# Borda/pyImSegm

Measured on NVIDIA H100. Metric: megapixels/sec end-to-end SLIC+features+GC (pipe_color2d_slic_features_model_graphcut), higher is better.
Workload: dtype f64

## Files before the change

pyimsegm_b200/csrc/graph.cu:

```cuda
#include "common.cuh"
#include <cooperative_groups.h>
namespace cg = cooperative_groups;

namespace {


struct AdjWs {
    unsigned long long* table;
    int* deg;
    int* off;
    int* fill;
    int* tmp_a;
    int* ctr;
    int slots;
};

__device__ __forceinline__ unsigned hash64(unsigned long long k)
{
    k ^= k >> 33; k *= 0xff51afd7ed558ccdull; k ^= k >> 33; k *= 0xc4ceb9fe1a85ec53ull; k ^= k >> 33;
    return (unsigned)k;
}

__device__ void edge_insert(const AdjWs& w, int l0, int l1)
{
// ... 160 lines not shown
    cg::cluster_group cl = cg::this_cluster();
    if (threadIdx.x == 0) *s_x = t;
    cl.sync();
    double tot = is_max ? -1.0 : 0.0;
    for (int r = 0; r < ECL; ++r) { const double pr = *cl.map_shared_rank(s_x, r); tot = is_max ? fmax(tot, pr) : tot + pr; }
    cl.sync();
    return tot;
}

__global__ void __cluster_dims__(ECL, 1, 1) __launch_bounds__(1024) k_gc_energies(const double* __restrict__ proba, int N_in, const int* n_nodes_dev, int K, const int* __restrict__ edges, int E_in,
                                                      const int* n_edges_dev, const double* __restrict__ centres,
                                                      const double* __restrict__ vfeat, int D, int metric, int spatial,
                                                      double edge_cost, const double* __restrict__ pairwise, double* unary,
                                                      double* edge_w, int* unary_i, int* edge_wi, int* smooth_i, double* sp)
{
    __shared__ double s_red[32];
    __shared__ double s_x;
    const int tid = blockIdx.x * blockDim.x + threadIdx.x, nth = gridDim.x * blockDim.x;
    const int E = n_edges_dev ? (*n_edges_dev > E_in ? 0 : *n_edges_dev) : E_in;
    const int N = n_nodes_dev ? min(*n_nodes_dev, N_in) : N_in;
    double umax = 0.0;
    for (int i = tid; i < N * K; i += nth) {
        double p = proba[i];
        if (p < 0.01) p = 0.01;
        if (p > 1.0 - 0.01) p = 1.0 - 0.01;
        double u = fabs(-log(p));
        unary[i] = u;
        umax = fmax(umax, fabs(u));
    }
    umax = cluster_reduce(umax, true, s_red, &s_x);
    double dsum = 0.0, ssum = 0.0;
    for (int e = tid; e < E; e += nth) {
        int a = edges[2 * e], b = edges[2 * e + 1];
        double dist = 0.0;
        if (metric != 0) {
            const double* va = vfeat + (size_t)a * D;
            const double* vb = vfeat + (size_t)b * D;
            for (int k = 0; k < D; ++k) {
                double df = va[k] - vb[k];
                if (metric == 1) dist = fmax(dist, df * df);
                else if (metric == 2) dist += fabs(df);
                else dist += df * df;
            }
            if (metric == 3) dist = sqrt(dist);
        }
        edge_w[e] = dist;
        dsum += dist;
        if (spatial) {
            double cy = centres[2 * a] - centres[2 * b], cx = centres[2 * a + 1] - centres[2 * b + 1];
            double s = sqrt(cy * cy + cx * cx);
            sp[e] = s;
            ssum += s;
        }
    }
    dsum = cluster_reduce(dsum, false, s_red, &s_x);
    ssum = cluster_reduce(ssum, false, s_red, &s_x);
    const double dmean = E > 0 ? dsum / E : 0.0, smean = E > 0 ? ssum / E : 1.0;
    double vsum = 0.0;
    if (metric != 0)
        for (int e = tid; e < E; e += nth) { double t = edge_w[e] - dmean; vsum += t * t; }
    vsum = cluster_reduce(vsum, false, s_red, &s_x);
    const double sd = sqrt(E > 0 ? vsum / E : 0.0);
    const double denom = 2.0 * (sd * sd);
    double wmax = 0.0;
    for (int e = tid; e < E; e += nth) {
        double wv = metric != 0 ? exp(-edge_w[e] / denom) : 1.0;
        if (spatial) wv = wv / (sp[e] / smean);
        if (wv < 1e-3) wv = 1e-3;
        if (wv > 1e3) wv = 1e3;
        wv *= edge_cost;
        edge_w[e] = wv;
        wmax = fmax(wmax, fabs(wv));
    }
    wmax = cluster_reduce(wmax, true, s_red, &s_x);
    double pmax = pairwise[0];
    for (int i = 1; i < K * K; ++i) pmax = fmax(pmax, pairwise[i]);
    const double dwf = fmax(umax, wmax * pmax) + 1e-10;
    for (int i = tid; i < N * K; i += nth) unary_i[i] = (int)((unary[i] / dwf) * 100000.0);
    for (int e = tid; e < E; e += nth) edge_wi[e] = (int)((edge_w[e] / dwf) * 1000.0);
    for (int i = tid; i < K * K; i += nth) smooth_i[i] = (int)(pairwise[i] * 100.0);
}


__global__ void __launch_bounds__(256) k_gather(const int* __restrict__ seg, long long n, const int* __restrict__ lut_i,
                                                const double* __restrict__ lut_p, int K, int* __restrict__ out_i, double* __restrict__ out_p)
{
    long long p = (long long)blockIdx.x * blockDim.x + threadIdx.x;
    if (p >= n) return;
    int l = seg[p];
    if (out_i) out_i[p] = lut_i[l];
    if (out_p) {
        const double* src = lut_p + (size_t)l * K;
        double* dst = out_p + (size_t)p * K;
        for (int k = 0; k < K; ++k) dst[k] = src[k];
    }
}

}

extern "C" size_t isb_adjacency_workspace_bytes(int nb, int cap)
{
    AdjWs w;
    return carve_adj(w, nullptr, 0, nb, cap);
}

extern "C" int isb_adjacency_edges(const int32_t* seg, int H, int W, int nb, int32_t* edges, int cap, int32_t* n_edges_out, void* ws,
                                   size_t ws_bytes, isb_stream_t stream)
{
    ISB_REQUIRE(seg && edges && n_edges_out && ws, "null pointer");
    ISB_REQUIRE(H > 0 && W > 0 && nb > 0 && cap > 0, "bad sizes");
    AdjWs w;
    size_t need = carve_adj(w, ws, ws_bytes, nb, cap);
    ISB_REQUIRE(need <= ws_bytes, "workspace too small");
    cudaStream_t st = (cudaStream_t)stream;
    ProfScope prof(ISB_PROF_ADJ, st);
    ISB_CUDA_CHECK(cudaMemsetAsync(w.table, 0xFF, sizeof(unsigned long long) * (size_t)w.slots, st));
    ISB_CUDA_CHECK(cudaMemsetAsync(w.deg, 0, sizeof(int) * (size_t)nb, st));
    ISB_CUDA_CHECK(cudaMemsetAsync(w.ctr, 0, sizeof(int) * 4, st));
    size_t n = (size_t)H * W;
    k_edge_scan<<<(unsigned)((n + 255) / 256), 256, 0, st>>>(seg, H, W, w);
    ISB_LAUNCH_CHECK();
    k_edge_offsets<<<1, 1024, 0, st>>>(nb, w, cap, n_edges_out);
    ISB_LAUNCH_CHECK();
    k_edge_fill<<<(w.slots + 255) / 256, 256, 0, st>>>(w, cap);
    ISB_LAUNCH_CHECK();
    k_edge_emit<<<(nb + 127) / 128, 128, 0, st>>>(nb, w, cap, edges);
    ISB_LAUNCH_CHECK();
    return ISB_OK;
}

extern "C" int isb_adjacency_edges_3d(const int32_t* seg, int D, int H, int W, int nb, int32_t* edges, int cap, int32_t* n_edges_out,
                                      void* ws, size_t ws_bytes, isb_stream_t stream)
{
    ISB_REQUIRE(seg && edges && n_edges_out && ws, "null pointer");
    ISB_REQUIRE(D > 0 && H > 0 && W > 0 && nb > 0 && cap > 0, "bad sizes");
    AdjWs w;
    size_t need = carve_adj(w, ws, ws_bytes, nb, cap);
    ISB_REQUIRE(need <= ws_bytes, "workspace too small");
    cudaStream_t st = (cudaStream_t)stream;
    ProfScope prof(ISB_PROF_ADJ, st);
    ISB_CUDA_CHECK(cudaMemsetAsync(w.table, 0xFF, sizeof(unsigned long long) * (size_t)w.slots, st));
    ISB_CUDA_CHECK(cudaMemsetAsync(w.deg, 0, sizeof(int) * (size_t)nb, st));
    ISB_CUDA_CHECK(cudaMemsetAsync(w.ctr, 0, sizeof(int) * 4, st));
    size_t n = (size_t)D * H * W;
    k_edge_scan3d<<<(unsigned)((n + 255) / 256), 256, 0, st>>>(seg, D, H, W, w);
    ISB_LAUNCH_CHECK();
    k_edge_offsets<<<1, 1024, 0, st>>>(nb, w, cap, n_edges_out);
    ISB_LAUNCH_CHECK();
    k_edge_fill<<<(w.slots + 255) / 256, 256, 0, st>>>(w, cap);
    ISB_LAUNCH_CHECK();
    k_edge_emit<<<(nb + 127) / 128, 128, 0, st>>>(nb, w, cap, edges);
    ISB_LAUNCH_CHECK();
    return ISB_OK;
}

extern "C" int isb_centroids_3d(const int32_t* seg, int D, int H, int W, int nb, double* centres, void* ws, size_t ws_bytes, isb_stream_t stream)
{
    ISB_REQUIRE(seg && centres && ws, "null pointer");
    ISB_REQUIRE(D > 0 && H > 0 && W > 0 && nb > 0, "bad sizes");
    ISB_REQUIRE(ws_bytes >= sizeof(unsigned long long) * 4 * (size_t)nb, "workspace too small (4 * nb uint64)");
    cudaStream_t st = (cudaStream_t)stream;
    ISB_CUDA_CHECK(cudaMemsetAsync(ws, 0, sizeof(unsigned long long) * 4 * (size_t)nb, st));
    size_t n = (size_t)D * H * W;
    k_centroid3d_acc<<<(unsigned)((n + 255) / 256), 256, 0, st>>>(seg, D, H, W, (unsigned long long*)ws);
    ISB_LAUNCH_CHECK();
    k_centroid3d_fin<<<(nb + 255) / 256, 256, 0, st>>>(nb, (const unsigned long long*)ws, centres);
    ISB_LAUNCH_CHECK();
    return ISB_OK;
}

extern "C" size_t isb_gc_energies_workspace_bytes(int N, int K, int E) { return isb_align(sizeof(double) * (size_t)(E > 0 ? E : 1)); }

extern "C" int isb_gc_energies(const double* proba, int N, const int32_t* n_nodes_dev, int K, const int32_t* edges, int E, const int32_t* n_edges_dev,
                               const double* centres, int metric, int spatial, double edge_cost, const double* pairwise, double* unary,
                               double* edge_w, int32_t* unary_i, int32_t* edge_wi, int32_t* smooth_i, void* ws, size_t ws_bytes,
                               isb_stream_t stream)
{
    ISB_REQUIRE(proba && edges && pairwise && unary && edge_w && unary_i && edge_wi && smooth_i && ws, "null pointer");
    ISB_REQUIRE(N > 0 && K > 0 && E >= 0, "bad sizes");
    ISB_REQUIRE(metric >= 0 && metric <= 3, "metric must be 0..3");
    ISB_REQUIRE(!spatial || centres, "centres are required for spatially normalised edge weights");
    ISB_REQUIRE(ws_bytes >= isb_gc_energies_workspace_bytes(N, K, E), "workspace too small");
    ProfScope prof(ISB_PROF_ENERGY, (cudaStream_t)stream);
    k_gc_energies<<<ECL, 1024, 0, (cudaStream_t)stream>>>(proba, N, n_nodes_dev, K, edges, E, n_edges_dev, centres, proba, K, metric, spatial, edge_cost,
                                                         pairwise, unary, edge_w, unary_i, edge_wi, smooth_i, (double*)ws);
    ISB_LAUNCH_CHECK();
    return ISB_OK;
}

__global__ void k_fill_i32(int* p, long long n, int v)
{
    long long i = (long long)blockIdx.x * blockDim.x + threadIdx.x;
    if (i < n) p[i] = v;
}

extern "C" int isb_fill_i32(int32_t* dst, long long n, int32_t value, isb_stream_t stream)
{
    ISB_REQUIRE(dst && n > 0, "bad arguments");
    k_fill_i32<<<(unsigned)((n + 255) / 256), 256, 0, (cudaStream_t)stream>>>(dst, n, value);
    ISB_LAUNCH_CHECK();
    return ISB_OK;
}

__global__ void k_combine(void* dst, const void* src, long long n, int op)
{
    long long i = (long long)blockIdx.x * blockDim.x + threadIdx.x;
    if (i >= n) return;
    if (op == 0) ((long long*)dst)[i] += ((const long long*)src)[i];
    else if (op == 1) { long long a = ((long long*)dst)[i], b = ((const long long*)src)[i]; ((long long*)dst)[i] = a > b ? a : b; }
    else if (op == 2) ((double*)dst)[i] = fmin(((double*)dst)[i], ((const double*)src)[i]);
    else if (op == 3) ((double*)dst)[i] = fmax(((double*)dst)[i], ((const double*)src)[i]);
    else ((double*)dst)[i] = ((double*)dst)[i] + ((const double*)src)[i];
}

extern "C" int isb_combine(void* dst, const void* src, long long n, int op, isb_stream_t stream)
{
    ISB_REQUIRE(dst && src && n > 0 && op >= 0 && op <= 4, "bad arguments");
    k_combine<<<(unsigned)((n + 255) / 256), 256, 0, (cudaStream_t)stream>>>(dst, src, n, op);
    ISB_LAUNCH_CHECK();
    return ISB_OK;
}

extern "C" int isb_gather(const int32_t* seg, long long npx, const int32_t* lut_i, const double* lut_p, int K, int32_t* out_i,
                          double* out_p, isb_stream_t stream)
{
    ISB_REQUIRE(seg && npx > 0, "bad arguments");
    ISB_REQUIRE((!out_i || lut_i) && (!out_p || (lut_p && K > 0)), "LUT missing for a requested output");
    ProfScope prof(ISB_PROF_GATHER, (cudaStream_t)stream);
    k_gather<<<(unsigned)((npx + 255) / 256), 256, 0, (cudaStream_t)stream>>>(seg, npx, lut_i, lut_p, K, out_i, out_p);
    ISB_LAUNCH_CHECK();
    return ISB_OK;
}
```

pyimsegm_b200/csrc/segment_stats.cu:

```cuda
#include "common.cuh"

namespace {

constexpr int SROWS = 16;

struct StatWs {
    double* acc;
    double* var;
    long long* iacc;
    float* meanf;
};

__device__ __forceinline__ float clean(float v) { return isnan(v) ? 0.0f : v; }

__global__ void __launch_bounds__(256) k_stats_pass1(const void* __restrict__ img, int dtype, const int* __restrict__ seg, int H, int W,
                                                     int y_off, StatWs ws)
{
    const int x = blockIdx.x * 256 + threadIdx.x;
    if (x >= W) return;
    const int y0 = blockIdx.y * SROWS, y1 = min(y0 + SROWS, H);
    int cur = -1;
    double s0 = 0, s1 = 0, s2 = 0, e0 = 0, e1 = 0, e2 = 0;
    long long cnt = 0, sy = 0;
    for (int y = y0; y <= y1; ++y) {
        int l = -1;
        float v0 = 0, v1 = 0, v2 = 0;
        if (y < y1) {
            size_t p = (size_t)y * W + x;
            l = seg[p];
            if (img) {
                v0 = clean(load_as_f32(img, dtype, 3 * p));
                v1 = clean(load_as_f32(img, dtype, 3 * p + 1));
                v2 = clean(load_as_f32(img, dtype, 3 * p + 2));
            }
        }
        if (l != cur) {
            if (cur >= 0) {
                double* a = ws.acc + 6 * (size_t)cur;
                atomicAdd(a, s0); atomicAdd(a + 1, s1); atomicAdd(a + 2, s2);
                atomicAdd(a + 3, e0); atomicAdd(a + 4, e1); atomicAdd(a + 5, e2);
                unsigned long long* ia = (unsigned long long*)(ws.iacc + 3 * (size_t)cur);
                atomicAdd(ia, (unsigned long long)cnt);
                atomicAdd(ia + 1, (unsigned long long)sy);
                atomicAdd(ia + 2, (unsigned long long)(cnt * x));
            }
            cur = l;
            s0 = s1 = s2 = e0 = e1 = e2 = 0;
            cnt = 0; sy = 0;
        }
        if (y < y1) {
            s0 += (double)v0; s1 += (double)v1; s2 += (double)v2;
            e0 += (double)__fmul_rn(v0, v0); e1 += (double)__fmul_rn(v1, v1); e2 += (double)__fmul_rn(v2, v2);
            cnt += 1; sy += y + y_off;
        }
    }
}

__global__ void k_stats_means(int nb, StatWs ws)
{
    int k = blockIdx.x * blockDim.x + threadIdx.x;
    if (k >= nb) return;
    long long c = ws.iacc[3 * (size_t)k];
    for (int z = 0; z < 3; ++z) {
        double m = ws.acc[6 * (size_t)k + z];
        if (c > 0) m = m / (double)c;
        ws.meanf[3 * (size_t)k + z] = (float)m;
    }
}

__global__ void __launch_bounds__(256) k_stats_pass2(const void* __restrict__ img, int dtype, const int* __restrict__ seg, int H, int W,
                                                     StatWs ws)
{
    const int x = blockIdx.x * 256 + threadIdx.x;
    if (x >= W) return;
    const int y0 = blockIdx.y * SROWS, y1 = min(y0 + SROWS, H);
    int cur = -1;
    double a0 = 0, a1 = 0, a2 = 0;
    float m0 = 0, m1 = 0, m2 = 0;
    for (int y = y0; y <= y1; ++y) {
        int l = -1;
        size_t p = (size_t)y * W + x;
        if (y < y1) l = seg[p];
        if (l != cur) {
            if (cur >= 0) {
                double* a = ws.var + 3 * (size_t)cur;
                atomicAdd(a, a0); atomicAdd(a + 1, a1); atomicAdd(a + 2, a2);
            }
            cur = l;
            a0 = a1 = a2 = 0;
            if (l >= 0) { m0 = ws.meanf[3 * (size_t)l]; m1 = ws.meanf[3 * (size_t)l + 1]; m2 = ws.meanf[3 * (size_t)l + 2]; }
        }
        if (y < y1) {
            float d0 = __fsub_rn(clean(load_as_f32(img, dtype, 3 * p)), m0);
            float d1 = __fsub_rn(clean(load_as_f32(img, dtype, 3 * p + 1)), m1);
            float d2 = __fsub_rn(clean(load_as_f32(img, dtype, 3 * p + 2)), m2);
            a0 += (double)__fmul_rn(d0, d0); a1 += (double)__fmul_rn(d1, d1); a2 += (double)__fmul_rn(d2, d2);
        }
    }
}

__device__ __forceinline__ double tidy(double v)
{
    if (isnan(v)) return 0.0;
    if (isinf(v)) return v > 0 ? 1.7976931348623157e308 : -1.7976931348623157e308;
    return v == 0.0 ? 0.0 : v;
}

__global__ void k_stats_finalize(int nb, int flags, StatWs ws, double* feat, int ld, int col0, double* centres, int* counts)
{
    int k = blockIdx.x * blockDim.x + threadIdx.x;
    if (k >= nb) return;
    long long c = ws.iacc[3 * (size_t)k];
    double dn = (double)c;
    int col = col0;
    double* row = feat ? feat + (size_t)k * ld : nullptr;
    if (row) {
        if (flags & 1) { for (int z = 0; z < 3; ++z) { double v = ws.acc[6 * (size_t)k + z]; if (c > 0) v = v / dn; row[col++] = tidy(v); } }
        if (flags & 2) { for (int z = 0; z < 3; ++z) { double v = ws.var[3 * (size_t)k + z]; if (c > 0) v = v / dn; row[col++] = tidy(sqrt(v)); } }
        if (flags & 4) { for (int z = 0; z < 3; ++z) { double v = ws.acc[6 * (size_t)k + 3 + z]; if (c > 0) v = v / dn; row[col++] = tidy(v); } }
    }
    if (centres) {
        if (c > 0) { centres[2 * (size_t)k] = (double)ws.iacc[3 * (size_t)k + 1] / dn; centres[2 * (size_t)k + 1] = (double)ws.iacc[3 * (size_t)k + 2] / dn; }
        else { centres[2 * (size_t)k] = -1.0; centres[2 * (size_t)k + 1] = -1.0; }
    }
    if (counts) counts[k] = (int)c;
}

static size_t carve(StatWs& w, void* ws, size_t bytes, int nb)
{
    WsCarver c(ws, bytes);
    w.acc = c.take<double>(6 * (size_t)nb);
    w.var = c.take<double>(3 * (size_t)nb);
    w.iacc = c.take<long long>(3 * (size_t)nb);
    w.meanf = c.take<float>(3 * (size_t)nb);
    return isb_align(c.off);
}

}

extern "C" size_t isb_segment_stats_workspace_bytes(int nb)
{
    StatWs w;
    return carve(w, nullptr, 0, nb);
}

extern "C" int isb_segment_stats_2d(const void* img, int dtype, const int32_t* seg, int H, int W, int nb, int flags, double* feat,
                                    int ld, int col0, double* centres, int32_t* counts, void* ws, size_t ws_bytes,
                                    isb_stream_t stream)
{
    ISB_REQUIRE(seg && ws && (img || (flags & 7) == 0), "null pointer");
    ISB_REQUIRE(H > 0 && W > 0 && nb > 0, "bad sizes");
    ISB_REQUIRE(dtype >= ISB_U8 && dtype <= ISB_F64, "bad dtype");
    StatWs w;
    size_t need = carve(w, ws, ws_bytes, nb);
    ISB_REQUIRE(need <= ws_bytes, "workspace too small");
    cudaStream_t st = (cudaStream_t)stream;
    ProfScope prof(ISB_PROF_STATS, st);
    ISB_CUDA_CHECK(cudaMemsetAsync(ws, 0, need, st));
    dim3 grid((W + 255) / 256, (H + SROWS - 1) / SROWS);
    k_stats_pass1<<<grid, 256, 0, st>>>(img, dtype, seg, H, W, 0, w);
    ISB_LAUNCH_CHECK();
    if (flags & 2) {
        k_stats_means<<<(nb + 255) / 256, 256, 0, st>>>(nb, w);
        ISB_LAUNCH_CHECK();
        k_stats_pass2<<<grid, 256, 0, st>>>(img, dtype, seg, H, W, w);
        ISB_LAUNCH_CHECK();
    }
    k_stats_finalize<<<(nb + 255) / 256, 256, 0, st>>>(nb, flags, w, feat, ld, col0, centres, counts);
    ISB_LAUNCH_CHECK();
    return ISB_OK;
}


extern "C" int isb_segment_stats_accumulate(const void* img, int dtype, const int32_t* seg, int H, int W, int y_off, int nb, double* acc,
                                            int64_t* iacc, isb_stream_t stream)
{
    ISB_REQUIRE(seg && acc && iacc, "null pointer");
    ISB_REQUIRE(H > 0 && W > 0 && nb > 0 && y_off >= 0, "bad sizes");
    ISB_REQUIRE(dtype >= ISB_U8 && dtype <= ISB_F64, "bad dtype");
    cudaStream_t st = (cudaStream_t)stream;
    ProfScope prof(ISB_PROF_STATS, st);
    StatWs w;
    w.acc = acc; w.iacc = (long long*)iacc; w.var = nullptr; w.meanf = nullptr;
    dim3 grid((W + 255) / 256, (H + SROWS - 1) / SROWS);
    k_stats_pass1<<<grid, 256, 0, st>>>(img, dtype, seg, H, W, y_off, w);
    ISB_LAUNCH_CHECK();
    return ISB_OK;
}

extern "C" int isb_segment_stats_deviation(const void* img, int dtype, const int32_t* seg, int H, int W, int nb, const double* acc,
                                           const int64_t* iacc, float* meanf_scratch, double* var, isb_stream_t stream)
{
    ISB_REQUIRE(img && seg && acc && iacc && meanf_scratch && var, "null pointer");
    ISB_REQUIRE(H > 0 && W > 0 && nb > 0, "bad sizes");
    ISB_REQUIRE(dtype >= ISB_U8 && dtype <= ISB_F64, "bad dtype");
    cudaStream_t st = (cudaStream_t)stream;
    ProfScope prof(ISB_PROF_STATS, st);
    StatWs w;
    w.acc = (double*)acc; w.iacc = (long long*)iacc; w.var = var; w.meanf = meanf_scratch;
    k_stats_means<<<(nb + 255) / 256, 256, 0, st>>>(nb, w);
    ISB_LAUNCH_CHECK();
    dim3 grid((W + 255) / 256, (H + SROWS - 1) / SROWS);
    k_stats_pass2<<<grid, 256, 0, st>>>(img, dtype, seg, H, W, w);
    ISB_LAUNCH_CHECK();
    return ISB_OK;
}

extern "C" int isb_segment_stats_finish(int nb, int flags, const double* acc, const double* var, const int64_t* iacc, double* feat, int ld,
                                        int col0, double* centres, int32_t* counts, isb_stream_t stream)
{
    ISB_REQUIRE(acc && iacc && (var || !(flags & 2)), "null pointer");
    ISB_REQUIRE(nb > 0, "bad sizes");
    cudaStream_t st = (cudaStream_t)stream;
    StatWs w;
    w.acc = (double*)acc; w.iacc = (long long*)iacc; w.var = (double*)var; w.meanf = nullptr;
    k_stats_finalize<<<(nb + 255) / 256, 256, 0, st>>>(nb, flags, w, feat, ld, col0, centres, counts);
    ISB_LAUNCH_CHECK();
    return ISB_OK;
}
```

pyimsegm_b200/csrc/slic_connectivity.cu:

```cuda
#include "common.cuh"

namespace {

struct ConnWs {
    int* comp;
    int* size;
    int* aux;
    int* queue;
    int* list;
    int* row_cnt;
    int* ctr;
    int4* bbox;
};

constexpr int VISBIT = 1 << 30;
__device__ __forceinline__ int dec(int c) { return (c < 0 ? ~c : c) & ~VISBIT; }

__device__ __forceinline__ int find_root(const int* parent, int i)
{
    while (true) {
        int p = parent[i];
        if (p == i) return i;
        i = p;
    }
}

__device__ __forceinline__ void unite(int* parent, int a, int b)
{
    while (true) {
        a = find_root(parent, a);
        b = find_root(parent, b);
        if (a == b) return;
        if (a < b) { int t = a; a = b; b = t; }
        int old = atomicMin(&parent[a], b);
        if (old == a) return;
        a = old;
    }
}

__global__ void __launch_bounds__(256) k_row_runs(const int* __restrict__ lab, int H, int W, int* __restrict__ parent)
{
    const int y = blockIdx.x;
    const int* row = lab + (size_t)y * W;
    int* prow = parent + (size_t)y * W;
    __shared__ int s_warp[8];
    __shared__ int s_carry;
    if (threadIdx.x == 0) s_carry = 0;
    __syncthreads();
    const int lane = threadIdx.x & 31, warp = threadIdx.x >> 5;
    for (int base = 0; base < W; base += 256) {
        int x = base + threadIdx.x;
        int v = -1;
        if (x < W) v = (x == 0 || row[x - 1] != row[x]) ? x : -1;
#pragma unroll
        for (int o = 1; o < 32; o <<= 1) {
            int t = __shfl_up_sync(0xffffffffu, v, o);
            if (lane >= o) v = max(v, t);
        }
        if (lane == 31) s_warp[warp] = v;
        __syncthreads();
        int pre = s_carry;
        for (int w = 0; w < warp; ++w) pre = max(pre, s_warp[w]);
        v = max(v, pre);
        if (x < W) prow[x] = y * W + v;
        __syncthreads();
        if (threadIdx.x == 255) s_carry = v;
        __syncthreads();
    }
}

__global__ void k_merge_vertical(const int* __restrict__ lab, int H, int W, int* parent)
{
    size_t p = (size_t)blockIdx.x * blockDim.x + threadIdx.x;
    if (p >= (size_t)H * W || p < (size_t)W) return;
    int x = (int)(p % W);
    int l = lab[p];
    if (lab[p - W] != l) return;
    if (x > 0 && lab[p - 1] == l && lab[p - W - 1] == l) return;
    unite(parent, (int)p, (int)(p - W));
}

__global__ void k_flatten_sizes(const int* __restrict__ lab, int H, int W, const int* __restrict__ parent, int* __restrict__ comp,
                                int* size)
{
    size_t p = (size_t)blockIdx.x * blockDim.x + threadIdx.x;
    if (p >= (size_t)H * W) return;
    int x = (int)(p % W);
    int rs = parent[p];
    int root = find_root(parent, rs);
    comp[p] = root;
    if (x == W - 1 || lab[p + 1] != lab[p]) {
        int xs = (x > 0 && lab[p - 1] == lab[p]) ? rs % W : x;
        atomicAdd(&size[root], x - xs + 1);
    }
}

__global__ void k_collect_oversize(int n, const int* __restrict__ comp, const int* __restrict__ size, int max_size, int* list,
                                   int* ctr, int* aux)
{
    int p = blockIdx.x * blockDim.x + threadIdx.x;
    if (p >= n) return;
    if (comp[p] == p && size[p] >= max_size) {
        int slot = atomicAdd(&ctr[0], 1);
        list[slot] = p;
        aux[p] = slot;
    }
}

__global__ void k_oversize_bbox(int H, int W, const int* __restrict__ comp, const int* __restrict__ size, int max_size,
                                const int* __restrict__ aux, const int* __restrict__ ctr, int4* bbox)
{
    if (ctr[0] == 0) return;
    size_t p = (size_t)blockIdx.x * blockDim.x + threadIdx.x;
    if (p >= (size_t)H * W) return;
    int r = comp[p];
    if (size[r] < max_size) return;
    int slot = aux[r];
    int y = (int)(p / W), x = (int)(p % W);
    atomicMin(&bbox[slot].x, y); atomicMax(&bbox[slot].y, y);
    atomicMin(&bbox[slot].z, x); atomicMax(&bbox[slot].w, x);
}

__global__ void k_oversize_split(int H, int W, int* comp, int* size, int max_size, const int* __restrict__ list,
                                 const int* __restrict__ ctr, const int4* __restrict__ bbox, int* queue)
{
    int i = blockIdx.x * blockDim.x + threadIdx.x;
    if (i >= ctr[0]) return;
    const int C = list[i];
    const int4 bb = bbox[i];
    int* q = queue + (size_t)i * max_size;
    const int total = size[C];
    int assigned = 0;
    for (int y = bb.x; y <= bb.y && assigned < total; ++y)
        for (int x = bb.z; x <= bb.w && assigned < total; ++x) {
            int p = y * W + x;
            if (comp[p] != C) continue;
            int start = p;
            comp[p] = ~start;
            q[0] = p;
            int n = 1, v = 0;
            while (v < n && n < max_size) {
                int cp = q[v];
                int cy = cp / W, cx = cp - cy * W;
                const int nx[4] = { cx + 1, cx - 1, cx, cx };
                const int ny[4] = { cy, cy, cy + 1, cy - 1 };
                for (int d = 0; d < 4; ++d) {
                    if (nx[d] < 0 || nx[d] >= W || ny[d] < 0 || ny[d] >= H) continue;
                    int np_ = ny[d] * W + nx[d];
                    if (comp[np_] == C) {
                        comp[np_] = ~start;
                        q[n++] = np_;
                        if (n >= max_size) break;
                    }
                }
                ++v;
            }
            size[start] = n;
            assigned += n;
        }
}

__global__ void __launch_bounds__(256) k_row_count_kept(int H, int W, const int* __restrict__ comp, const int* __restrict__ size,
                                                        int min_size, int* row_cnt)
{
    const int y = blockIdx.x;
    int c = 0;
    for (int x = threadIdx.x; x < W; x += 256) {
        int p = y * W + x;
        c += (dec(comp[p]) == p && size[p] >= min_size) ? 1 : 0;
    }
    __shared__ int s[256];
    s[threadIdx.x] = c;
    __syncthreads();
    for (int o = 128; o > 0; o >>= 1) {
        if (threadIdx.x < o) s[threadIdx.x] += s[threadIdx.x + o];
        __syncthreads();
    }
    if (threadIdx.x == 0) row_cnt[y] = s[0];
}

__global__ void __launch_bounds__(1024) k_scan_rows(int H, int* row_cnt, int* n_labels_out)
{
    __shared__ int s_part[1024];
    __shared__ int s_carry;
    if (threadIdx.x == 0) s_carry = 0;
    __syncthreads();
    for (int base = 0; base < H; base += 1024) {
        int i = base + threadIdx.x;
        int v = i < H ? row_cnt[i] : 0;
        s_part[threadIdx.x] = v;
        __syncthreads();
        for (int o = 1; o < 1024; o <<= 1) {
            int t = threadIdx.x >= o ? s_part[threadIdx.x - o] : 0;
            __syncthreads();
            s_part[threadIdx.x] += t;
            __syncthreads();
        }
        int incl = s_part[threadIdx.x], carry = s_carry;
        if (i < H) row_cnt[i] = carry + incl - v;
        __syncthreads();
        if (threadIdx.x == 1023) s_carry = carry + incl;
        __syncthreads();
    }
// ... 42 lines not shown
        q[0] = C;
        comp[C] = (comp[C] < 0 ? ~(dec(comp[C]) | VISBIT) : (comp[C] | VISBIT));
        int n = 1, v = 0;
        while (v < n && n < max_size) {
            const int cp = q[v * QS];
            const int cy = cp / W, cx = cp - cy * W;
            const int np4[4] = { cx + 1 < W ? cp + 1 : -1, cx > 0 ? cp - 1 : -1, cy + 1 < H ? cp + W : -1, cy > 0 ? cp - W : -1 };
            int raw4[4];
#pragma unroll
            for (int d = 0; d < 4; ++d) raw4[d] = np4[d] >= 0 ? comp[np4[d]] : 0;
#pragma unroll
            for (int d = 0; d < 4; ++d) {
                if (np4[d] < 0) continue;
                const int raw = raw4[d];
                const int r = dec(raw);
                if (r == C) {
                    const bool seen = ((raw < 0 ? ~raw : raw) & VISBIT) != 0;
                    if (!seen) {
                        comp[np4[d]] = raw < 0 ? ~((~raw) | VISBIT) : (raw | VISBIT);
                        q[(n++) * QS] = np4[d];
                        if (n >= max_size) break;
                    }
                } else if (r < C) {
                    adjacent = r;
                }
            }
            ++v;
        }
        aux[C] = adjacent >= 0 ? -2 - adjacent : -1;
    }
}

__global__ void k_write_labels(int n, const int* __restrict__ comp, const int* __restrict__ size, int min_size,
                               const int* __restrict__ aux, int* __restrict__ out)
{
    int p = blockIdx.x * blockDim.x + threadIdx.x;
    if (p >= n) return;
    int r = dec(comp[p]);
    int a = aux[r];
    while (a < -1) { r = -2 - a; a = aux[r]; }
    out[p] = a < 0 ? 0 : a;
}

static size_t carve(ConnWs& w, void* ws, size_t bytes, int H, int W)
{
    WsCarver c(ws, bytes);
    size_t n = (size_t)H * W;
    w.comp = c.take<int>(n); w.size = c.take<int>(n); w.aux = c.take<int>(n);
    w.queue = c.take<int>(n); w.list = c.take<int>(n);
    w.row_cnt = c.take<int>((size_t)H + 1);
    w.ctr = c.take<int>(8);
    w.bbox = c.take<int4>(n / 16 + 16);
    return isb_align(c.off);
}

__global__ void k_init_bbox(int n, int4* bbox)
{
    int i = blockIdx.x * blockDim.x + threadIdx.x;
    if (i < n) bbox[i] = make_int4(INT_MAX, -1, INT_MAX, -1);
}

}

extern "C" size_t isb_connectivity_workspace_bytes(int H, int W)
{
    ConnWs w;
    return carve(w, nullptr, 0, H, W);
}

extern "C" int isb_enforce_connectivity(const int32_t* labels, int H, int W, int min_size, int max_size, int32_t* out,
                                        int32_t* n_labels_out, void* ws, size_t ws_bytes, isb_stream_t stream)
{
    ISB_REQUIRE(labels && out && n_labels_out && ws, "null pointer");
    ISB_REQUIRE(H > 0 && W > 0 && (long long)H * W < (1LL << 30), "bad image size (at most 2^30 pixels)");
    if (max_size < 1) max_size = 1;
    ISB_REQUIRE(max_size >= 16, "max_size < 16 is not supported on the device path (oversize table bound)");
    ConnWs w;
    size_t need = carve(w, ws, ws_bytes, H, W);
    ISB_REQUIRE(need <= ws_bytes, "workspace too small");
    cudaStream_t st = (cudaStream_t)stream;
    ProfScope prof(ISB_PROF_CONN, st);
    const int n = H * W;
    const int nb = (n + 255) / 256;
    ISB_CUDA_CHECK(cudaMemsetAsync(w.size, 0, sizeof(int) * (size_t)n, st));
    ISB_CUDA_CHECK(cudaMemsetAsync(w.ctr, 0, sizeof(int) * 8, st));
    k_row_runs<<<H, 256, 0, st>>>(labels, H, W, w.comp);
    ISB_LAUNCH_CHECK();
    k_merge_vertical<<<nb, 256, 0, st>>>(labels, H, W, w.comp);
    ISB_LAUNCH_CHECK();
    k_flatten_sizes<<<nb, 256, 0, st>>>(labels, H, W, w.comp, w.aux, w.size);
    ISB_LAUNCH_CHECK();
    int* comp = w.aux;
    int* aux = w.comp;
    const int n_over_max = n / max_size + 1;
    k_init_bbox<<<(n_over_max + 255) / 256, 256, 0, st>>>(n_over_max, w.bbox);
    ISB_LAUNCH_CHECK();
    k_collect_oversize<<<nb, 256, 0, st>>>(n, comp, w.size, max_size, w.list, w.ctr, aux);
    ISB_LAUNCH_CHECK();
    k_oversize_bbox<<<nb, 256, 0, st>>>(H, W, comp, w.size, max_size, aux, w.ctr, w.bbox);
    ISB_LAUNCH_CHECK();
    k_oversize_split<<<(n_over_max + 63) / 64, 64, 0, st>>>(H, W, comp, w.size, max_size, w.list, w.ctr, w.bbox, w.queue);
    ISB_LAUNCH_CHECK();
    k_row_count_kept<<<H, 256, 0, st>>>(H, W, comp, w.size, min_size, w.row_cnt);
    ISB_LAUNCH_CHECK();
    k_scan_rows<<<1, 1024, 0, st>>>(H, w.row_cnt, n_labels_out);
    ISB_LAUNCH_CHECK();
    k_row_assign_labels<<<H, 256, 0, st>>>(H, W, comp, w.size, min_size, w.row_cnt, aux, w.list, w.ctr);
    ISB_LAUNCH_CHECK();
    {
        int dev = 0, sms = 0;
        ISB_CUDA_CHECK(cudaGetDevice(&dev));
        ISB_CUDA_CHECK(cudaDeviceGetAttribute(&sms, cudaDevAttrMultiProcessorCount, dev));
        if (min_size >= 1 && min_size <= 512) {
            const size_t smem = sizeof(int) * 32 * (size_t)min_size;
            ISB_CUDA_CHECK(cudaFuncSetAttribute(k_small_adjacent<true>, cudaFuncAttributeMaxDynamicSharedMemorySize, (int)smem));
            k_small_adjacent<true><<<sms * 16, 32, smem, st>>>(H, W, comp, w.size, max_size, w.list, w.ctr, aux, w.queue);
        } else {
            k_small_adjacent<false><<<sms * 8, 256, 0, st>>>(H, W, comp, w.size, max_size, w.list, w.ctr, aux, w.queue);
        }
        ISB_LAUNCH_CHECK();
    }
    k_write_labels<<<nb, 256, 0, st>>>(n, comp, w.size, min_size, aux, out);
    ISB_LAUNCH_CHECK();
    return ISB_OK;
}
```

Before: 1481.

## Tile-local CCL, shared-memory segment stat aggregation, and vectorized gather

```diff
diff --git a/pyimsegm_b200/csrc/graph.cu b/pyimsegm_b200/csrc/graph.cu
--- a/pyimsegm_b200/csrc/graph.cu
+++ b/pyimsegm_b200/csrc/graph.cu
@@ -266,12 +266,37 @@
 }
 
 
-__global__ void __launch_bounds__(256) k_gather(const int* __restrict__ seg, long long n, const int* __restrict__ lut_i,
-                                                const double* __restrict__ lut_p, int K, int* __restrict__ out_i, double* __restrict__ out_p)
-{
-    long long p = (long long)blockIdx.x * blockDim.x + threadIdx.x;
+constexpr int GW = 128;
+
+__global__ void __launch_bounds__(256) k_gather(const int* __restrict__ seg, long long n, long long head, long long n_warp,
+                                                const int* __restrict__ lut_i, const double* __restrict__ lut_p, int K,
+                                                int* __restrict__ out_i, double* __restrict__ out_p)
+{
+    __shared__ int s_lab[256 / 32][GW];
+    const long long t = (long long)blockIdx.x * blockDim.x + threadIdx.x;
+    const long long gw = t >> 5;
+    const int lane = threadIdx.x & 31;
+    if (gw < n_warp) {
+        const long long base = head + gw * GW;
+        const int4 l4 = *reinterpret_cast<const int4*>(seg + base + 4 * lane);
+        if (out_i)
+            *reinterpret_cast<int4*>(out_i + base + 4 * lane) = make_int4(__ldg(lut_i + l4.x), __ldg(lut_i + l4.y), __ldg(lut_i + l4.z), __ldg(lut_i + l4.w));
+        if (out_p) {
+            int* sl = s_lab[threadIdx.x >> 5];
+            *reinterpret_cast<int4*>(sl + 4 * lane) = l4;
+            __syncwarp();
+            double2* dst = reinterpret_cast<double2*>(out_p + base * K);
+            for (int i = lane; i < GW * K / 2; i += 32) {
+                const int e = 2 * i, q0 = e / K, c0 = e - q0 * K, q1 = (e + 1) / K, c1 = e + 1 - q1 * K;
+                dst[i] = make_double2(__ldg(lut_p + (size_t)sl[q0] * K + c0), __ldg(lut_p + (size_t)sl[q1] * K + c1));
+            }
+        }
+        return;
+    }
+    const long long j = t - n_warp * 32;
+    const long long p = j < head ? j : j + n_warp * GW;
     if (p >= n) return;
-    int l = seg[p];
+    const int l = seg[p];
     if (out_i) out_i[p] = lut_i[l];
     if (out_p) {
         const double* src = lut_p + (size_t)l * K;
@@ -411,7 +436,12 @@
     ISB_REQUIRE(seg && npx > 0, "bad arguments");
     ISB_REQUIRE((!out_i || lut_i) && (!out_p || (lut_p && K > 0)), "LUT missing for a requested output");
     ProfScope prof(ISB_PROF_GATHER, (cudaStream_t)stream);
-    k_gather<<<(unsigned)((npx + 255) / 256), 256, 0, (cudaStream_t)stream>>>(seg, npx, lut_i, lut_p, K, out_i, out_p);
-    ISB_LAUNCH_CHECK();
-    return ISB_OK;
-}
+    const long long head = (long long)((16 - ((uintptr_t)seg & 15)) & 15) / 4;
+    const bool aligned = head < npx && (!out_i || ((uintptr_t)(out_i + head) & 15) == 0) && (!out_p || ((uintptr_t)(out_p + head * K) & 15) == 0);
+    const long long n_warp = aligned ? (npx - head) / GW : 0;
+    const long long n_thr = n_warp * 32 + (npx - n_warp * GW);
+    k_gather<<<(unsigned)((n_thr + 255) / 256), 256, 0, (cudaStream_t)stream>>>(seg, npx, aligned ? head : 0, n_warp, lut_i, lut_p, K, out_i,
+                                                                                  out_p);
+    ISB_LAUNCH_CHECK();
+    return ISB_OK;
+}
diff --git a/pyimsegm_b200/csrc/segment_stats.cu b/pyimsegm_b200/csrc/segment_stats.cu
--- a/pyimsegm_b200/csrc/segment_stats.cu
+++ b/pyimsegm_b200/csrc/segment_stats.cu
@@ -2,7 +2,7 @@
 
 namespace {
 
-constexpr int SROWS = 16;
+constexpr int SROWS = 32;
 
 struct StatWs {
     double* acc;
@@ -13,46 +13,172 @@
 
 __device__ __forceinline__ float clean(float v) { return isnan(v) ? 0.0f : v; }
 
-__global__ void __launch_bounds__(256) k_stats_pass1(const void* __restrict__ img, int dtype, const int* __restrict__ seg, int H, int W,
-                                                     int y_off, StatWs ws)
-{
-    const int x = blockIdx.x * 256 + threadIdx.x;
-    if (x >= W) return;
-    const int y0 = blockIdx.y * SROWS, y1 = min(y0 + SROWS, H);
-    int cur = -1;
-    double s0 = 0, s1 = 0, s2 = 0, e0 = 0, e1 = 0, e2 = 0;
-    long long cnt = 0, sy = 0;
-    for (int y = y0; y <= y1; ++y) {
-        int l = -1;
-        float v0 = 0, v1 = 0, v2 = 0;
-        if (y < y1) {
-            size_t p = (size_t)y * W + x;
-            l = seg[p];
-            if (img) {
-                v0 = clean(load_as_f32(img, dtype, 3 * p));
-                v1 = clean(load_as_f32(img, dtype, 3 * p + 1));
-                v2 = clean(load_as_f32(img, dtype, 3 * p + 2));
-            }
-        }
-        if (l != cur) {
-            if (cur >= 0) {
-                double* a = ws.acc + 6 * (size_t)cur;
-                atomicAdd(a, s0); atomicAdd(a + 1, s1); atomicAdd(a + 2, s2);
-                atomicAdd(a + 3, e0); atomicAdd(a + 4, e1); atomicAdd(a + 5, e2);
-                unsigned long long* ia = (unsigned long long*)(ws.iacc + 3 * (size_t)cur);
-                atomicAdd(ia, (unsigned long long)cnt);
-                atomicAdd(ia + 1, (unsigned long long)sy);
-                atomicAdd(ia + 2, (unsigned long long)(cnt * x));
-            }
-            cur = l;
-            s0 = s1 = s2 = e0 = e1 = e2 = 0;
-            cnt = 0; sy = 0;
-        }
-        if (y < y1) {
-            s0 += (double)v0; s1 += (double)v1; s2 += (double)v2;
-            e0 += (double)__fmul_rn(v0, v0); e1 += (double)__fmul_rn(v1, v1); e2 += (double)__fmul_rn(v2, v2);
-            cnt += 1; sy += y + y_off;
-        }
+template <int MODE> struct StatMode {
+    static constexpr int ND = MODE == 0 ? 0 : (MODE == 1 ? 6 : 3);
+    static constexpr int NQ = MODE == 2 ? 0 : 3;
+};
+
+template <int MODE>
+__device__ __forceinline__ void add_global(const StatWs& ws, int key, const double* d, const long long* q)
+{
+    if (MODE == 1) { double* a = ws.acc + 6 * (size_t)key; for (int i = 0; i < 6; ++i) atomicAdd(a + i, d[i]); }
+    if (MODE == 2) { double* a = ws.var + 3 * (size_t)key; for (int i = 0; i < 3; ++i) atomicAdd(a + i, d[i]); }
+    if (MODE != 2) {
+        unsigned long long* ia = (unsigned long long*)(ws.iacc + 3 * (size_t)key);
+        for (int i = 0; i < 3; ++i) atomicAdd(ia + i, (unsigned long long)q[i]);
+    }
+}
+
+template <int ND, int NQ>
+__device__ __forceinline__ bool warp_segment_sum(bool fl, int key, double* d, long long* q)
+{
+    const unsigned FULL = 0xffffffffu;
+    const int lane = threadIdx.x & 31;
+    const unsigned fm = __ballot_sync(FULL, fl);
+    const int kprev = __shfl_up_sync(FULL, key, 1);
+    const bool head = fl && !(lane > 0 && ((fm >> (lane - 1)) & 1u) && kprev == key);
+    const unsigned heads = __ballot_sync(FULL, head);
+    const unsigned stop = (heads | ~fm) & ~((2u << lane) - 1u);
+    const int end = stop ? __ffs(stop) - 2 : 31;
+#pragma unroll
+    for (int o = 1; o < 32; o <<= 1) {
+        const bool take = lane + o <= end;
+#pragma unroll
+        for (int i = 0; i < ND; ++i) { const double t = __shfl_down_sync(FULL, d[i], o); if (take) d[i] += t; }
+#pragma unroll
+        for (int i = 0; i < NQ; ++i) { const long long t = __shfl_down_sync(FULL, q[i], o); if (take) q[i] += t; }
+    }
+    return head;
+}
+
+constexpr int RUNS = 3, TS = 64;
+
+template <typename T, int MODE>
+__global__ void __launch_bounds__(256) k_stats_tile(const T* __restrict__ img, const int* __restrict__ seg, int H, int W, int y_off,
+                                                    StatWs ws)
+{
+    constexpr int ND = StatMode<MODE>::ND, NQ = StatMode<MODE>::NQ, NDS = ND > 0 ? ND : 1, NQS = NQ > 0 ? NQ : 1;
+    __shared__ int s_key[TS];
+    __shared__ double s_td[TS][NDS];
+    __shared__ unsigned long long s_tq[TS][NQS];
+    __shared__ int s_rl[RUNS][256];
+    __shared__ int s_rc[RUNS][256];
+    __shared__ double s_rd[RUNS][NDS][256];
+    const int tid = threadIdx.x, x = blockIdx.x * 256 + tid, y0 = blockIdx.y * SROWS;
+    const int n = x < W ? min(SROWS, H - y0) : 0;
+    for (int i = tid; i < TS; i += 256) {
+        s_key[i] = -1;
+        for (int k = 0; k < NDS; ++k) s_td[i][k] = 0;
+        for (int k = 0; k < NQS; ++k) s_tq[i][k] = 0;
+    }
+    const long long ybase = (long long)y0 + y_off;
+    int cur = -1, nrun = 0, cnt = 0, syl = 0;
+    double a[NDS];
+#pragma unroll
+    for (int k = 0; k < NDS; ++k) a[k] = 0;
+    float m0 = 0, m1 = 0, m2 = 0;
+    auto end_run = [&]() {
+        if (nrun < RUNS) {
+            s_rl[nrun][tid] = cur;
+            s_rc[nrun][tid] = cnt | (syl << 8);
+#pragma unroll
+            for (int k = 0; k < ND; ++k) s_rd[nrun][k][tid] = a[k];
+        } else {
+            const long long q[3] = { cnt, cnt * ybase + syl, (long long)cnt * x };
+            add_global<MODE>(ws, cur, a, q);
+        }
+        ++nrun;
+    };
+    constexpr int B = 8;
+    for (int rb = 0; rb < SROWS; rb += B) {
+        int lb[B];
+        float vb[B][3];
+#pragma unroll
+        for (int k = 0; k < B; ++k) {
+            lb[k] = -1;
+            vb[k][0] = vb[k][1] = vb[k][2] = 0.0f;
+            if (rb + k < n) {
+                const size_t p = (size_t)(y0 + rb + k) * W + x;
+                lb[k] = seg[p];
+                if (MODE != 0) {
+                    vb[k][0] = clean((float)img[3 * p]);
+                    vb[k][1] = clean((float)img[3 * p + 1]);
+                    vb[k][2] = clean((float)img[3 * p + 2]);
+                }
+            }
+        }
+#pragma unroll
+        for (int k = 0; k < B; ++k) {
+            if (rb + k >= n) break;
+            const int l = lb[k];
+            if (l != cur) {
+                if (cur >= 0) end_run();
+                cur = l; cnt = 0; syl = 0;
+#pragma unroll
+                for (int i = 0; i < NDS; ++i) a[i] = 0;
+                if (MODE == 2 && l >= 0) { m0 = ws.meanf[3 * (size_t)l]; m1 = ws.meanf[3 * (size_t)l + 1]; m2 = ws.meanf[3 * (size_t)l + 2]; }
+            }
+            const float v0 = vb[k][0], v1 = vb[k][1], v2 = vb[k][2];
+            if (MODE == 1) {
+                a[0] += (double)v0; a[1] += (double)v1; a[2] += (double)v2;
+                a[3] += (double)__fmul_rn(v0, v0); a[4] += (double)__fmul_rn(v1, v1); a[5] += (double)__fmul_rn(v2, v2);
+            }
+            if (MODE == 2) {
+                const float d0 = __fsub_rn(v0, m0), d1 = __fsub_rn(v1, m1), d2 = __fsub_rn(v2, m2);
+                a[0] += (double)__fmul_rn(d0, d0); a[1] += (double)__fmul_rn(d1, d1); a[2] += (double)__fmul_rn(d2, d2);
+            }
+            cnt += 1; syl += rb + k;
+        }
+    }
+    if (cur >= 0) end_run();
+    __syncthreads();
+    for (int r = 0; r < RUNS; ++r) {
+        const bool has = r < nrun;
+        if (!__any_sync(0xffffffffu, has)) break;
+        int key = -1;
+        double d[NDS];
+        long long q[NQS];
+#pragma unroll
+        for (int k = 0; k < NDS; ++k) d[k] = 0;
+#pragma unroll
+        for (int k = 0; k < NQS; ++k) q[k] = 0;
+        if (has) {
+            key = s_rl[r][tid];
+#pragma unroll
+            for (int k = 0; k < ND; ++k) d[k] = s_rd[r][k][tid];
+            if constexpr (NQ > 0) {
+                const int c = s_rc[r][tid] & 0xff, sl = s_rc[r][tid] >> 8;
+                q[0] = c; q[1] = c * ybase + sl; q[2] = (long long)c * x;
+            }
+        }
+        if (warp_segment_sum<ND, NQ>(has, key, d, q)) {
+            unsigned h = ((unsigned)key * 2654435761u) >> 26;
+            int slot = -1;
+            for (int probe = 0; probe < TS; ++probe, h = (h + 1) & (TS - 1)) {
+                const int old = atomicCAS(&s_key[h], -1, key);
+                if (old == -1 || old == key) { slot = (int)h; break; }
+            }
+            if (slot < 0) {
+                add_global<MODE>(ws, key, d, q);
+            } else {
+#pragma unroll
+                for (int k = 0; k < ND; ++k) atomicAdd(&s_td[slot][k], d[k]);
+#pragma unroll
+                for (int k = 0; k < NQ; ++k) atomicAdd(&s_tq[slot][k], (unsigned long long)q[k]);
+            }
+        }
+    }
+    __syncthreads();
+    for (int i = tid; i < TS; i += 256) {
+        const int key = s_key[i];
+        if (key < 0) continue;
+        double d[NDS];
+        long long q[NQS];
+#pragma unroll
+        for (int k = 0; k < NDS; ++k) d[k] = s_td[i][k];
+#pragma unroll
+        for (int k = 0; k < NQS; ++k) q[k] = (long long)s_tq[i][k];
+        add_global<MODE>(ws, key, d, q);
     }
 }
 
@@ -65,37 +191,6 @@
         double m = ws.acc[6 * (size_t)k + z];
         if (c > 0) m = m / (double)c;
         ws.meanf[3 * (size_t)k + z] = (float)m;
-    }
-}
-
-__global__ void __launch_bounds__(256) k_stats_pass2(const void* __restrict__ img, int dtype, const int* __restrict__ seg, int H, int W,
-                                                     StatWs ws)
-{
-    const int x = blockIdx.x * 256 + threadIdx.x;
-    if (x >= W) return;
-    const int y0 = blockIdx.y * SROWS, y1 = min(y0 + SROWS, H);
-    int cur = -1;
-    double a0 = 0, a1 = 0, a2 = 0;
-    float m0 = 0, m1 = 0, m2 = 0;
-    for (int y = y0; y <= y1; ++y) {
-        int l = -1;
-        size_t p = (size_t)y * W + x;
-        if (y < y1) l = seg[p];
-        if (l != cur) {
-            if (cur >= 0) {
-                double* a = ws.var + 3 * (size_t)cur;
-                atomicAdd(a, a0); atomicAdd(a + 1, a1); atomicAdd(a + 2, a2);
-            }
-            cur = l;
-            a0 = a1 = a2 = 0;
-            if (l >= 0) { m0 = ws.meanf[3 * (size_t)l]; m1 = ws.meanf[3 * (size_t)l + 1]; m2 = ws.meanf[3 * (size_t)l + 2]; }
-        }
-        if (y < y1) {
-            float d0 = __fsub_rn(clean(load_as_f32(img, dtype, 3 * p)), m0);
-            float d1 = __fsub_rn(clean(load_as_f32(img, dtype, 3 * p + 1)), m1);
-            float d2 = __fsub_rn(clean(load_as_f32(img, dtype, 3 * p + 2)), m2);
-            a0 += (double)__fmul_rn(d0, d0); a1 += (double)__fmul_rn(d1, d1); a2 += (double)__fmul_rn(d2, d2);
-        }
     }
 }
 
@@ -126,6 +221,27 @@
     if (counts) counts[k] = (int)c;
 }
 
+template <typename T>
+static void launch_tile_t(const void* img, int mode, const int* seg, int H, int W, int y_off, const StatWs& w, cudaStream_t st)
+{
+    const dim3 grid((W + 255) / 256, (H + SROWS - 1) / SROWS);
+    const T* im = (const T*)img;
+    if (mode == 0) k_stats_tile<T, 0><<<grid, 256, 0, st>>>(im, seg, H, W, y_off, w);
+    else if (mode == 1) k_stats_tile<T, 1><<<grid, 256, 0, st>>>(im, seg, H, W, y_off, w);
+    else k_stats_tile<T, 2><<<grid, 256, 0, st>>>(im, seg, H, W, y_off, w);
+}
+
+static void launch_tile(const void* img, int dtype, int mode, const int* seg, int H, int W, int y_off, const StatWs& w, cudaStream_t st)
+{
+    if (mode == 0) { launch_tile_t<unsigned char>(nullptr, 0, seg, H, W, y_off, w, st); return; }
+    switch (dtype) {
+        case ISB_U8: launch_tile_t<unsigned char>(img, mode, seg, H, W, y_off, w, st); break;
+        case ISB_U16: launch_tile_t<unsigned short>(img, mode, seg, H, W, y_off, w, st); break;
+        case ISB_F32: launch_tile_t<float>(img, mode, seg, H, W, y_off, w, st); break;
+        default: launch_tile_t<double>(img, mode, seg, H, W, y_off, w, st); break;
+    }
+}
+
 static size_t carve(StatWs& w, void* ws, size_t bytes, int nb)
 {
     WsCarver c(ws, bytes);
@@ -157,13 +273,12 @@
     cudaStream_t st = (cudaStream_t)stream;
     ProfScope prof(ISB_PROF_STATS, st);
     ISB_CUDA_CHECK(cudaMemsetAsync(ws, 0, need, st));
-    dim3 grid((W + 255) / 256, (H + SROWS - 1) / SROWS);
-    k_stats_pass1<<<grid, 256, 0, st>>>(img, dtype, seg, H, W, 0, w);
+    launch_tile(img, dtype, img ? 1 : 0, seg, H, W, 0, w, st);
     ISB_LAUNCH_CHECK();
     if (flags & 2) {
         k_stats_means<<<(nb + 255) / 256, 256, 0, st>>>(nb, w);
         ISB_LAUNCH_CHECK();
-        k_stats_pass2<<<grid, 256, 0, st>>>(img, dtype, seg, H, W, w);
+        launch_tile(img, dtype, 2, seg, H, W, 0, w, st);
         ISB_LAUNCH_CHECK();
     }
     k_stats_finalize<<<(nb + 255) / 256, 256, 0, st>>>(nb, flags, w, feat, ld, col0, centres, counts);
@@ -182,8 +297,7 @@
     ProfScope prof(ISB_PROF_STATS, st);
     StatWs w;
     w.acc = acc; w.iacc = (long long*)iacc; w.var = nullptr; w.meanf = nullptr;
-    dim3 grid((W + 255) / 256, (H + SROWS - 1) / SROWS);
-    k_stats_pass1<<<grid, 256, 0, st>>>(img, dtype, seg, H, W, y_off, w);
+    launch_tile(img, dtype, img ? 1 : 0, seg, H, W, y_off, w, st);
     ISB_LAUNCH_CHECK();
     return ISB_OK;
 }
@@ -200,8 +314,7 @@
     w.acc = (double*)acc; w.iacc = (long long*)iacc; w.var = var; w.meanf = meanf_scratch;
     k_stats_means<<<(nb + 255) / 256, 256, 0, st>>>(nb, w);
     ISB_LAUNCH_CHECK();
-    dim3 grid((W + 255) / 256, (H + SROWS - 1) / SROWS);
-    k_stats_pass2<<<grid, 256, 0, st>>>(img, dtype, seg, H, W, w);
+    launch_tile(img, dtype, 2, seg, H, W, 0, w, st);
     ISB_LAUNCH_CHECK();
     return ISB_OK;
 }
diff --git a/pyimsegm_b200/csrc/slic_connectivity.cu b/pyimsegm_b200/csrc/slic_connectivity.cu
--- a/pyimsegm_b200/csrc/slic_connectivity.cu
+++ b/pyimsegm_b200/csrc/slic_connectivity.cu
@@ -38,72 +38,128 @@
     }
 }
 
-__global__ void __launch_bounds__(256) k_row_runs(const int* __restrict__ lab, int H, int W, int* __restrict__ parent)
-{
-    const int y = blockIdx.x;
-    const int* row = lab + (size_t)y * W;
-    int* prow = parent + (size_t)y * W;
-    __shared__ int s_warp[8];
-    __shared__ int s_carry;
-    if (threadIdx.x == 0) s_carry = 0;
-    __syncthreads();
-    const int lane = threadIdx.x & 31, warp = threadIdx.x >> 5;
-    for (int base = 0; base < W; base += 256) {
-        int x = base + threadIdx.x;
-        int v = -1;
-        if (x < W) v = (x == 0 || row[x - 1] != row[x]) ? x : -1;
-#pragma unroll
-        for (int o = 1; o < 32; o <<= 1) {
-            int t = __shfl_up_sync(0xffffffffu, v, o);
-            if (lane >= o) v = max(v, t);
+constexpr int TH = 32, TW = 64, TPX = TH * TW;
+
+__device__ __forceinline__ int find_root_s(const volatile int* par, int i)
+{
+    while (true) {
+        const int p = par[i];
+        if (p == i) return i;
+        i = p;
+    }
+}
+
+__device__ __forceinline__ void unite_s(int* par, int a, int b)
+{
+    while (true) {
+        a = find_root_s(par, a);
+        b = find_root_s(par, b);
+        if (a == b) return;
+        if (a < b) { const int t = a; a = b; b = t; }
+        const int old = atomicMin(&par[a], b);
+        if (old == a) return;
+        a = old;
+    }
+}
+
+__global__ void __launch_bounds__(256) k_tile_ccl(const int* __restrict__ lab, int H, int W, int* __restrict__ parent, int* __restrict__ size)
+{
+    __shared__ int s_lab[TPX];
+    __shared__ int s_par[TPX];
+    const int tx0 = blockIdx.x * TW, ty0 = blockIdx.y * TH;
+    const int vw = min(TW, W - tx0), vh = min(TH, H - ty0);
+    const int x = threadIdx.x & (TW - 1), lane = threadIdx.x & 31;
+    constexpr int RSTEP = 256 / TW, NR = TH / RSTEP;
+#pragma unroll
+    for (int k = 0; k < NR; ++k) {
+        const int y = (threadIdx.x / TW) + RSTEP * k;
+        s_lab[y * TW + x] = (x < vw && y < vh) ? lab[(size_t)(ty0 + y) * W + tx0 + x] : 0;
+    }
+    __syncthreads();
+#pragma unroll
+    for (int k = 0; k < NR; ++k) {
+        const int y = (threadIdx.x / TW) + RSTEP * k, i = y * TW + x;
+        const bool join_left = x > 0 && x < vw && s_lab[i - 1] == s_lab[i];
+        const unsigned m = __ballot_sync(0xffffffffu, !join_left) & ((2u << lane) - 1u);
+        s_par[i] = m ? i - lane + (31 - __clz(m)) : i - lane - 1;
+    }
+    __syncthreads();
+#pragma unroll
+    for (int k = 0; k < NR; ++k) {
+        const int y = (threadIdx.x / TW) + RSTEP * k, i = y * TW + x;
+        if (x >= vw || y >= vh || y == 0) continue;
+        const int l = s_lab[i];
+        if (s_lab[i - TW] != l) continue;
+        if (x > 0 && s_lab[i - 1] == l && s_lab[i - TW - 1] == l) continue;
+        unite_s(s_par, i, i - TW);
+    }
+    __syncthreads();
+    int root[NR];
+#pragma unroll
+    for (int k = 0; k < NR; ++k) {
+        const int y = (threadIdx.x / TW) + RSTEP * k, i = y * TW + x;
+        root[k] = find_root_s(s_par, i);
+        s_lab[i] = 0;
+    }
+    __syncthreads();
+#pragma unroll
+    for (int k = 0; k < NR; ++k) {
+        const int y = (threadIdx.x / TW) + RSTEP * k;
+        if (x < vw && y < vh) atomicAdd(&s_lab[root[k]], 1);
+    }
+    __syncthreads();
+#pragma unroll
+    for (int k = 0; k < NR; ++k) {
+        const int y = (threadIdx.x / TW) + RSTEP * k, i = y * TW + x;
+        if (x >= vw || y >= vh) continue;
+        const size_t p = (size_t)(ty0 + y) * W + tx0 + x;
+        parent[p] = (ty0 + root[k] / TW) * W + tx0 + root[k] % TW;
+        size[p] = root[k] == i ? s_lab[i] : 0;
+    }
+}
+
+__global__ void k_seam_merge(const int* __restrict__ lab, int H, int W, int* parent)
+{
+    const long long t = (long long)blockIdx.x * blockDim.x + threadIdx.x;
+    const long long n_up = (long long)((H - 1) / TH) * W;
+    if (t < n_up) {
+        const int y = (int)(t / W + 1) * TH, x = (int)(t % W);
+        const int p = y * W + x, l = lab[p];
+        if (lab[p - W] != l) return;
+        if (x % TW != 0 && lab[p - 1] == l && lab[p - W - 1] == l) return;
+        unite(parent, p, p - W);
+        return;
+    }
+    const long long u = t - n_up;
+    if (u >= (long long)((W - 1) / TW) * H) return;
+    const int x = (int)(u / H + 1) * TW, y = (int)(u % H);
+    const int p = y * W + x, l = lab[p];
+    if (lab[p - 1] != l) return;
+    if (y % TH != 0 && lab[p - W] == l && lab[p - W - 1] == l) return;
+    unite(parent, p, p - 1);
+}
+
+__global__ void k_flatten(int n, const int* __restrict__ parent, int* __restrict__ comp, int* size, int* roots, int* ctr)
+{
+    const int p = blockIdx.x * blockDim.x + threadIdx.x;
+    if (p >= n) return;
+    const int r = find_root(parent, parent[p]);
+    comp[p] = r;
+    if (r == p) { roots[atomicAdd(&ctr[3], 1)] = p; return; }
+    const int s = size[p];
+    if (s > 0) atomicAdd(&size[r], s);
+}
+
+__global__ void k_collect_oversize(const int* __restrict__ roots, const int* __restrict__ size, int max_size, int* list, int* ctr, int* aux)
+{
+    const int n_roots = ctr[3];
+    for (int i = blockIdx.x * blockDim.x + threadIdx.x; i < n_roots; i += gridDim.x * blockDim.x) {
+        const int p = roots[i];
+        if (size[p] >= max_size) {
+            const int slot = atomicAdd(&ctr[0], 1);
+            list[slot] = p;
+            aux[p] = slot;
         }
-        if (lane == 31) s_warp[warp] = v;
-        __syncthreads();
-        int pre = s_carry;
-        for (int w = 0; w < warp; ++w) pre = max(pre, s_warp[w]);
-        v = max(v, pre);
-        if (x < W) prow[x] = y * W + v;
-        __syncthreads();
-        if (threadIdx.x == 255) s_carry = v;
-        __syncthreads();
-    }
-}
-
-__global__ void k_merge_vertical(const int* __restrict__ lab, int H, int W, int* parent)
-{
-    size_t p = (size_t)blockIdx.x * blockDim.x + threadIdx.x;
-    if (p >= (size_t)H * W || p < (size_t)W) return;
-    int x = (int)(p % W);
-    int l = lab[p];
-    if (lab[p - W] != l) return;
-    if (x > 0 && lab[p - 1] == l && lab[p - W - 1] == l) return;
-    unite(parent, (int)p, (int)(p - W));
-}
-
-__global__ void k_flatten_sizes(const int* __restrict__ lab, int H, int W, const int* __restrict__ parent, int* __restrict__ comp,
-                                int* size)
-{
-    size_t p = (size_t)blockIdx.x * blockDim.x + threadIdx.x;
-    if (p >= (size_t)H * W) return;
-    int x = (int)(p % W);
-    int rs = parent[p];
-    int root = find_root(parent, rs);
-    comp[p] = root;
-    if (x == W - 1 || lab[p + 1] != lab[p]) {
-        int xs = (x > 0 && lab[p - 1] == lab[p]) ? rs % W : x;
-        atomicAdd(&size[root], x - xs + 1);
-    }
-}
-
-__global__ void k_collect_oversize(int n, const int* __restrict__ comp, const int* __restrict__ size, int max_size, int* list,
-                                   int* ctr, int* aux)
-{
-    int p = blockIdx.x * blockDim.x + threadIdx.x;
-    if (p >= n) return;
-    if (comp[p] == p && size[p] >= max_size) {
-        int slot = atomicAdd(&ctr[0], 1);
-        list[slot] = p;
-        aux[p] = slot;
     }
 }
 
@@ -111,14 +167,14 @@
                                 const int* __restrict__ aux, const int* __restrict__ ctr, int4* bbox)
 {
     if (ctr[0] == 0) return;
-    size_t p = (size_t)blockIdx.x * blockDim.x + threadIdx.x;
-    if (p >= (size_t)H * W) return;
-    int r = comp[p];
-    if (size[r] < max_size) return;
-    int slot = aux[r];
-    int y = (int)(p / W), x = (int)(p % W);
-    atomicMin(&bbox[slot].x, y); atomicMax(&bbox[slot].y, y);
-    atomicMin(&bbox[slot].z, x); atomicMax(&bbox[slot].w, x);
+    for (size_t p = (size_t)blockIdx.x * blockDim.x + threadIdx.x; p < (size_t)H * W; p += (size_t)gridDim.x * blockDim.x) {
+        const int r = comp[p];
+        if (size[r] < max_size) continue;
+        const int slot = aux[r];
+        const int y = (int)(p / W), x = (int)(p % W);
+        atomicMin(&bbox[slot].x, y); atomicMax(&bbox[slot].y, y);
+        atomicMin(&bbox[slot].z, x); atomicMax(&bbox[slot].w, x);
+    }
 }
 
 __global__ void k_oversize_split(int H, int W, int* comp, int* size, int max_size, const int* __restrict__ list,
@@ -327,22 +383,27 @@
     ProfScope prof(ISB_PROF_CONN, st);
     const int n = H * W;
     const int nb = (n + 255) / 256;
-    ISB_CUDA_CHECK(cudaMemsetAsync(w.size, 0, sizeof(int) * (size_t)n, st));
+    int dev = 0, sms = 0;
+    ISB_CUDA_CHECK(cudaGetDevice(&dev));
+    ISB_CUDA_CHECK(cudaDeviceGetAttribute(&sms, cudaDevAttrMultiProcessorCount, dev));
     ISB_CUDA_CHECK(cudaMemsetAsync(w.ctr, 0, sizeof(int) * 8, st));
-    k_row_runs<<<H, 256, 0, st>>>(labels, H, W, w.comp);
-    ISB_LAUNCH_CHECK();
-    k_merge_vertical<<<nb, 256, 0, st>>>(labels, H, W, w.comp);
-    ISB_LAUNCH_CHECK();
-    k_flatten_sizes<<<nb, 256, 0, st>>>(labels, H, W, w.comp, w.aux, w.size);
+    k_tile_ccl<<<dim3((W + TW - 1) / TW, (H + TH - 1) / TH), 256, 0, st>>>(labels, H, W, w.comp, w.size);
+    ISB_LAUNCH_CHECK();
+    {
+        const long long n_seam = (long long)((H - 1) / TH) * W + (long long)((W - 1) / TW) * H;
+        if (n_seam > 0) k_seam_merge<<<(unsigned)((n_seam + 255) / 256), 256, 0, st>>>(labels, H, W, w.comp);
+        ISB_LAUNCH_CHECK();
+    }
+    k_flatten<<<nb, 256, 0, st>>>(n, w.comp, w.aux, w.size, w.queue, w.ctr);
     ISB_LAUNCH_CHECK();
     int* comp = w.aux;
     int* aux = w.comp;
     const int n_over_max = n / max_size + 1;
     k_init_bbox<<<(n_over_max + 255) / 256, 256, 0, st>>>(n_over_max, w.bbox);
     ISB_LAUNCH_CHECK();
-    k_collect_oversize<<<nb, 256, 0, st>>>(n, comp, w.size, max_size, w.list, w.ctr, aux);
-    ISB_LAUNCH_CHECK();
-    k_oversize_bbox<<<nb, 256, 0, st>>>(H, W, comp, w.size, max_size, aux, w.ctr, w.bbox);
+    k_collect_oversize<<<sms * 4, 256, 0, st>>>(w.queue, w.size, max_size, w.list, w.ctr, aux);
+    ISB_LAUNCH_CHECK();
+    k_oversize_bbox<<<sms * 4, 256, 0, st>>>(H, W, comp, w.size, max_size, aux, w.ctr, w.bbox);
     ISB_LAUNCH_CHECK();
     k_oversize_split<<<(n_over_max + 63) / 64, 64, 0, st>>>(H, W, comp, w.size, max_size, w.list, w.ctr, w.bbox, w.queue);
     ISB_LAUNCH_CHECK();
@@ -353,9 +414,6 @@
     k_row_assign_labels<<<H, 256, 0, st>>>(H, W, comp, w.size, min_size, w.row_cnt, aux, w.list, w.ctr);
     ISB_LAUNCH_CHECK();
     {
-        int dev = 0, sms = 0;
-        ISB_CUDA_CHECK(cudaGetDevice(&dev));
-        ISB_CUDA_CHECK(cudaDeviceGetAttribute(&sms, cudaDevAttrMultiProcessorCount, dev));
         if (min_size >= 1 && min_size <= 512) {
             const size_t smem = sizeof(int) * 32 * (size_t)min_size;
             ISB_CUDA_CHECK(cudaFuncSetAttribute(k_small_adjacent<true>, cudaFuncAttributeMaxDynamicSharedMemorySize, (int)smem));
```

Measured after the change: 1541, median of 6. 4.0% higher.
